# Stanford-ILIAD/PantheonRL

Hardware: AMD Instinct MI355X
Metric: env-steps/sec (all agents) Overcooked-simple PPO self-play (higher is better)
Workload: dtype f32; 1 GPU; OvercookedMultiEnv-v0 layout=simple, PPO self-play (two independent PPO learners per GPU), synthetic (n_envs, n_steps, obs_dim) rollouts; n_envs=1024, n_steps=128, obs_dim=62, features=62, n_logits=6, batch_size=32768, n_epochs=10, agents_per_gpu=2, parallelism=2 agent(s) per gpu x1 gpu(s) = 2 learners (single process), launch_mode=graph, gemm_mode=2, action_masks=none, rollout=scripted, rollout_requested=scripted

## Files before the change

include/pantheon_hip.h:

```cpp
#ifndef PANTHEON_HIP_H
#define PANTHEON_HIP_H

#ifdef __cplusplus
extern "C" {
#endif

#define PH_ABI_VERSION 7
#define PH_HIDDEN 64
#define PH_MAX_COMP 256
#define PH_MAX_LOGITS 64
#define PH_MAX_BOX_ACT 16
#define PH_NSTAT 8
#define PH_MOD_MAX 8
#define PH_MAX_RANKS 16

#define PH_SPACE_BOX 0
#define PH_SPACE_DISCRETE 1

typedef struct ph_ctx ph_ctx;

typedef struct ph_space {
  int kind;
  int n;
  int nvec[PH_MAX_COMP];
// ... 8 lines not shown
  int D;
  int F;
  int A;
  int L;
  int P;
  int pi_W1, pi_b1, pi_W2, pi_b2, vf_W1, vf_b1, vf_W2, vf_b2, act_W, act_b, val_W, val_b;
} ph_layout;

typedef struct ph_rollout {
  int T, E;
  float *observations;
  float *actions;
  float *rewards;
  float *episode_starts;
  float *values;
  float *log_probs;
  float *advantages;
  float *returns;
} ph_rollout;

typedef struct ph_ppo_hyper {
  float learning_rate;
  float clip_range;
  float clip_range_vf;
  float ent_coef;
  float vf_coef;
  float max_grad_norm;
  float target_kl;
  int normalize_advantage;
  float adam_beta1, adam_beta2, adam_eps;
} ph_ppo_hyper;

typedef struct ph_opt_state {
  float *params;
  float *adam_m;
  float *adam_v;
  int *step;
} ph_opt_state;

int ph_abi_version(void);
const char *ph_last_error(void);
int ph_device_count(int *n_out );
int ph_ctx_create(int device, ph_ctx **out );
int ph_ctx_destroy(ph_ctx *ctx);
int ph_ctx_set_stream(ph_ctx *ctx, void *hip_stream );
int ph_ctx_sync(ph_ctx *ctx);
int ph_graph_begin(ph_ctx *ctx);
int ph_graph_end(ph_ctx *ctx, int *graph_id_out );
int ph_graph_launch(ph_ctx *ctx, int graph_id);
int ph_ctx_set_rng_epoch(ph_ctx *ctx, unsigned long long *epoch_dev );
int ph_rng_epoch_advance(ph_ctx *ctx);
int ph_debug_set_profile_buffer(ph_ctx *ctx, long long *stamps_dev);
int ph_debug_weight_image_mismatches(ph_ctx *ctx, const ph_spec *spec, const float *params, int *mismatches);
int ph_set_exclusive_device(ph_ctx *ctx, int exclusive);
int ph_ctx_step_errors(ph_ctx *ctx, unsigned int *count_out );
int ph_timer_start(ph_ctx *ctx);
int ph_timer_stop(ph_ctx *ctx, float *ms_out );

int ph_layout_of(const ph_spec *spec , ph_layout *out );
int ph_debug_split_tables(const ph_spec *spec, int *slab_map, int *image_map, int *eligible);
int ph_debug_split_oh_tables(const ph_spec *spec, int *slab_map, int *image_map, int *slab_len_out, int *image_elems_out,
                             int *eligible);

int ph_buffer_add(ph_ctx *ctx, const ph_spec *spec, const ph_rollout *rb, int pos, const float *obs ,
                  const float *actions , const float *episode_start ,
                  const float *values , const float *log_probs );
int ph_buffer_add_reward(ph_ctx *ctx, const ph_rollout *rb, int pos, const float *reward ,
                         const unsigned char *env_mask );
int ph_buffer_add_reward_const(ph_ctx *ctx, const ph_rollout *rb, int pos, float reward);
#define PH_JOINT_MATCH_BONUS 0
#define PH_JOINT_RPS 1
int ph_ctx_set_joint_reward_rule(ph_ctx *ctx, int rule);

int ph_buffer_add_reward_joint(ph_ctx *ctx, const ph_rollout *rb, int pos, const float *base_reward ,
                               const int *joint_actions, int n_seats, int seat, const int *partner_seat ,
                               float bonus);
int ph_roundrobin_env_step(ph_ctx *ctx, const int *joint_actions, int *partnerid, const float *base_reward,
                           const float *done, float *reward_out, int *alt_action_out, float *next_block, int block_ld,
                           int n_partners, float bonus, int n);
typedef struct ph_rr_link {
  int n_partners, rank;
  int n, block_ld;
  void *area[PH_MAX_RANKS];
  unsigned long long *error;
  unsigned long long timeout_cycles;
} ph_rr_link;
typedef struct ph_rr_ego {
  const ph_spec *spec;
  const float *params;
  const float *obs_seq;
  const float *base_reward_seq;
  const float *done_seq;
  float *blocks;
  int *partnerid;
  float *rewards;
  int *alt_actions;
  int *partner_trace;
  const float *episode_start0;
  unsigned long long seed, counter0;
  float *values, *log_probs;
  const ph_rollout *rb;
  float bonus;
} ph_rr_ego;
typedef struct ph_rr_partner {
  const ph_spec *spec;
  const float *params;
// ... 458 lines not shown
```

pantheonrl_amd/_native.py:

```python
from __future__ import annotations

import ctypes as C
import os
from typing import Optional, Sequence

PH_HIDDEN = 64
PH_MAX_COMP = 256
PH_MAX_LOGITS = 64
PH_MAX_BOX_ACT = 16
PH_NSTAT = 8
PH_SPACE_BOX = 0
PH_SPACE_DISCRETE = 1
STAT_NAMES = ("policy_loss", "value_loss", "entropy_loss", "clip_fraction", "approx_kl", "loss", "grad_norm", "applied")

_HERE = os.path.dirname(os.path.abspath(__file__))
LIB_PATH = os.environ.get("PANTHEON_HIP_LIB") or os.path.join(_HERE, "csrc", "libpantheon_hip.so")


class NativeError(RuntimeError):
    """Raised for any non-zero status from the C ABI (message from ph_last_error)."""


class PhSpace(C.Structure):
    _fields_ = [("kind", C.c_int), ("n", C.c_int), ("nvec", C.c_int * PH_MAX_COMP)]
# ... 160 lines not shown
                ("alt_values", C.c_void_p), ("alt_log_probs", C.c_void_p), ("alt_pos", C.c_void_p),
                ("alt_boundary", C.c_void_p), ("alt_term", C.c_void_p), ("alt_open", C.c_void_p), ("alt_acted", C.c_void_p),
                ("alt_seed", C.c_ulonglong),
                ("obs_ego", C.c_void_p), ("obs_alt", C.c_void_p), ("episodes", C.c_void_p),
                ("es_alt", C.c_void_p), ("running", C.c_void_p), ("can", C.c_void_p), ("done", C.c_void_p)]


PH_BLOCK_STATE_WORDS = 12

PH_MAX_POOL = 8
PH_POOL_LEARNER, PH_POOL_FROZEN, PH_POOL_SCRIPTED = 0, 1, 2
POOL_RESAMPLE = {"robin": 0, "random": 1}


class PhPoolMember(C.Structure):
    _fields_ = [("kind", C.c_int), ("params", C.c_void_p), ("rb", C.POINTER(PhRollout)), ("pos", C.c_void_p),
                ("boundary", C.c_void_p), ("term", C.c_void_p), ("open", C.c_void_p), ("values", C.c_void_p),
                ("log_probs", C.c_void_p), ("seed", C.c_ulonglong)]


class PhLiarPool(C.Structure):
    _fields_ = [("n", C.c_int), ("spec", C.POINTER(PhSpec)),
                ("hands", C.c_void_p), ("history", C.c_void_p), ("nmoves", C.c_void_p), ("ego_first", C.c_void_p),
                ("dice_seed", C.c_ulonglong), ("probegostart", C.c_float),
                ("ego_params", C.c_void_p), ("ego_rb", C.POINTER(PhRollout)), ("ego_actions", C.c_void_p),
                ("ego_values", C.c_void_p), ("ego_log_probs", C.c_void_p), ("ego_episode_start", C.c_void_p),
                ("ego_seed", C.c_ulonglong),
                ("members", C.POINTER(PhPoolMember)), ("n_members", C.c_int), ("partnerid", C.c_void_p),
                ("resample", C.c_int), ("pool_seed", C.c_ulonglong),
                ("alt_actions", C.c_void_p), ("alt_acted", C.c_void_p),
                ("obs_ego", C.c_void_p), ("obs_alt", C.c_void_p), ("episodes", C.c_void_p),
                ("obs_next", C.c_void_p), ("rew1", C.c_void_p), ("rew2", C.c_void_p), ("es_alt", C.c_void_p),
                ("done1", C.c_void_p), ("done2", C.c_void_p), ("running", C.c_void_p), ("can", C.c_void_p),
                ("alt_opens", C.c_void_p), ("ego_opens", C.c_void_p), ("done", C.c_void_p)]

SIGNATURES = {
    "ph_abi_version": [],
    "ph_roundrobin_env_step": [_vp, _vp, _vp, _vp, _vp, _vp, _vp, _vp, _i, _i, C.c_float, _i],
    "ph_last_error": [],
    "ph_device_count": [C.POINTER(_i)],
    "ph_ctx_create": [_i, C.POINTER(_vp)],
    "ph_ctx_destroy": [_vp],
    "ph_ctx_set_stream": [_vp, _vp],
    "ph_ctx_sync": [_vp],
    "ph_graph_begin": [_vp],
    "ph_graph_end": [_vp, C.POINTER(_i)],
    "ph_graph_launch": [_vp, _i],
    "ph_ctx_set_rng_epoch": [_vp, _vp],
    "ph_rng_epoch_advance": [_vp],
    "ph_debug_set_profile_buffer": [_vp, _vp],
    "ph_set_exclusive_device": [_vp, _i],
    "ph_ctx_step_errors": [_vp, C.POINTER(C.c_uint)],
    "ph_debug_weight_image_mismatches": [_vp, C.POINTER(PhSpec), _vp, C.POINTER(C.c_int)],
    "ph_timer_start": [_vp],
    "ph_timer_stop": [_vp, C.POINTER(C.c_float)],
    "ph_layout_of": [C.POINTER(PhSpec), C.POINTER(PhLayout)],
    "ph_debug_split_tables": [C.POINTER(PhSpec), C.POINTER(C.c_int), C.POINTER(C.c_int), C.POINTER(C.c_int)],
    "ph_debug_split_oh_tables": [C.POINTER(PhSpec), _vp, _vp, C.POINTER(_i), C.POINTER(_i), C.POINTER(_i)],
    "ph_buffer_add": [_vp, C.POINTER(PhSpec), C.POINTER(PhRollout), _i, _vp, _vp, _vp, _vp, _vp],
    "ph_buffer_add_reward": [_vp, C.POINTER(PhRollout), _i, _vp, _vp],
    "ph_buffer_add_reward_joint": [_vp, C.POINTER(PhRollout), _i, _vp, _vp, _i, _i, _vp, C.c_float],
    "ph_buffer_reset": [_vp, C.POINTER(PhSpec), C.POINTER(PhRollout)],
    "ph_gae": [_vp, C.POINTER(PhRollout), _vp, _vp, _d, _d, _i],
    "ph_policy_forward": [_vp, C.POINTER(PhSpec), _vp, _vp, _i, _vp, _vp, _vp, _ull, _ull, _i, _vp, _vp, _vp, _vp, _vp,
                          _vp, C.POINTER(PhRollout), _i, _vp, _vp, _i],
    "ph_ctx_set_joint_reward_rule": [_vp, _i],
    "ph_adapmult_layout_of": [C.POINTER(PhSpec), _i, _vp],
    "ph_adapmult_forward": [_vp, C.POINTER(PhSpec), _i, _vp, _vp, _i, _vp, _vp, _vp, _ull, _ull, _i, _vp, _vp, _vp, _vp, _vp,
                            _vp, C.POINTER(PhRollout), _i, _vp],
    "ph_adapmult_minibatch_grad": [_vp, C.POINTER(PhSpec), _i, _vp, C.POINTER(PhRollout), C.POINTER(PhPpoHyper), _vp, _i, _vp, _vp,
                                   _vp],
    "ph_adapmult_train": [_vp, C.POINTER(PhSpec), _i, C.POINTER(PhOptState), C.POINTER(PhRollout), C.POINTER(PhPpoHyper), _i, _i,
                          _vp, _ull, _vp, _vp],
    "ph_policy_act_host": [_vp, C.POINTER(PhSpec), _vp, _vp, _i, _vp, _ull, _ull, _i, _vp, _vp, _vp, C.POINTER(PhRollout), _i, _i],
    "ph_buffer_add_reward_const": [_vp, C.POINTER(PhRollout), _i, C.c_float],
    "ph_policy_step_multi": [_vp, _i, C.POINTER(PhStepCall)],
    "ph_policy_forward_ragged": [_vp, C.POINTER(PhSpec), _vp, _vp, _vp, _ull, _ull, _i, _vp, _vp, _vp, C.POINTER(PhRollout),
                                 _vp, _vp, _vp],
    "ph_buffer_add_reward_ragged": [_vp, C.POINTER(PhRollout), _vp, _vp, _vp],
    "ph_ragged_advance": [_vp, C.POINTER(PhRollout), _vp, _vp],
    "ph_buffer_compact_columns": [_vp, C.POINTER(PhSpec), C.POINTER(PhRollout), C.POINTER(PhRollout), _vp, _i],
    "ph_fix_illegal_actions": [_vp, _vp, _vp, _i, _i],
    "ph_rps_step": [_vp, _vp, _vp, _vp, _vp, _i],
    "ph_liar_step": [_vp, _vp, _vp, _vp, _vp, _vp, _vp, _vp, _vp, _vp, _i],
    "ph_liar_reset": [_vp, _vp, _vp, _vp, _vp, _vp, _ull, _ull, C.c_float, _i],
    "ph_liar_obs": [_vp, _vp, _vp, _vp, _vp, _vp, _vp, _i],
    "ph_liar_selfplay_step": [_vp, C.POINTER(PhLiarSelfPlay), _i, _ull, _i],
    "ph_liar_selfplay_rollout": [_vp, C.POINTER(PhLiarSelfPlay), _i, _i, _ull],
    "ph_pool_forward": [_vp, C.POINTER(PhSpec), C.POINTER(PhPoolMember), _i, _vp, _vp, _vp, _ull, _vp, _vp, _i],
    "ph_liar_default_actions": [_vp, _vp, _vp, _vp, _i],
    "ph_liar_pool_step": [_vp, C.POINTER(PhLiarPool), _i, _ull, _i],
    "ph_block_reset": [_vp, _i, _vp, _vp, _ull, _ull, _i],
    "ph_block_step": [_vp, _i, _vp, _vp, _i, _vp, _vp, _vp, _vp, _i],
    "ph_block_obs": [_vp, _i, _vp, _i, _vp, _vp, _i],
    "ph_block_selfplay_step": [_vp, C.POINTER(PhBlockSelfPlay), _i, _ull],
    "ph_block_replay_host": [_i, _i, _i, _vp, _vp, _vp, _vp, _vp, _vp, _vp, _i, _ull, _ull, _i],
    "ph_framestack_push": [_vp, _vp, _vp, _vp, _vp, _i, _i, _i],
    "ph_scripted_rollout": [_vp, C.POINTER(PhSpec), _vp, _vp, _vp, _vp, _i, _i, _vp, _ull, _ull, _vp, _vp, _vp,
                            C.POINTER(PhRollout), _i, _i],
    "ph_ppo_train": [_vp, C.POINTER(PhSpec), C.POINTER(PhOptState), C.POINTER(PhRollout), C.POINTER(PhPpoHyper), _i, _i,
                     _vp, _ull, _vp, _i],
    "ph_ppo_train_multi": [C.POINTER(PhTrainCall), _i],
    "ph_comm_unique_id": [_vp],
    "ph_comm_init": [_vp, _vp, _i, _i],
    "ph_comm_destroy": [_vp],
    "ph_all_gather_i32": [_vp, _vp, _vp, _i],
# ... 233 lines not shown
```

pantheonrl_amd/csrc/ph_abi.hip:

```cpp
#include <dlfcn.h>
#include <hip/hip_runtime.h>
#include <rccl/rccl.h>

#include <atomic>
#include <chrono>
#include <cmath>
#include <cstdio>
#include <cstdint>
#include <cstring>
#include <mutex>
#include <string>
#include <vector>

#include "ph_launch.h"
#include "ph_block.h"
#include "ph_arch.h"
#include "ph_pool.h"

namespace ph {

namespace {
struct LdsGrant {
  const void* kernel;
  int device;
// ... 75 lines not shown
}

struct ph_ctx {
  int device = 0;
  hipStream_t stream = nullptr;
  float* slabs = nullptr;
  size_t slabs_cap = 0;
  float* statpart = nullptr;
  size_t statpart_cap = 0;
  float* grad = nullptr;
  size_t grad_cap = 0;
  float* blocksq = nullptr;
  size_t blocksq_cap = 0;
  float* advstats = nullptr;
  size_t advstats_cap = 0;
  ph::AdamBias* adam_bias = nullptr;
  size_t adam_bias_cap = 0;
  float* act_stage_host = nullptr;
  float* act_stage_dev = nullptr;
  size_t act_stage_cap = 0;
  unsigned int* act_done_host = nullptr;
  unsigned int* act_done_dev = nullptr;
  unsigned int act_seq = 0;
  unsigned int* fwd_host_done = nullptr;
  int joint_reward_rule = 0;
  int wimage_zeroed_for = 0;
  size_t wimage_cap = 0;
  bool exclusive = false;
  unsigned short* wimage = nullptr;
  double* advpart = nullptr;
  size_t advpart_cap = 0;
  int* perm_idx = nullptr;
  size_t perm_idx_cap = 0;
  int* perm_phys = nullptr;
  size_t perm_phys_cap = 0;
  uint4* ximg = nullptr;
  size_t ximg_cap = 0;
  uint4* rec_pi = nullptr;
  uint4* rec_vf = nullptr;
  size_t rec_cap = 0;
  uint4* rowrec = nullptr;
  size_t rowrec_cap = 0;
  unsigned long long* step_words = nullptr;
  size_t step_words_cap = 0;
  unsigned int* step_gen = nullptr;
  float* am_buf = nullptr;
  size_t am_buf_cap = 0;
  float* adap_extra = nullptr;
  size_t adap_extra_cap = 0;
  float* adap_loss = nullptr;
  size_t adap_loss_cap = 0;
  float* scalars = nullptr;
  int* stop_flag = nullptr;
  std::vector<SpecCache> specs;
  std::vector<hipGraphExec_t> graphs;
  bool capturing = false;
  hipEvent_t ev0 = nullptr, ev1 = nullptr;
  ph_p2p* p2p_dev = nullptr;
  ph_p2p p2p_host;
  bool p2p_valid = false;
  void* comm = nullptr;
  int comm_world = 1, comm_rank = 0;
  hipEvent_t ev_grad = nullptr;
  int num_cu = 256;
  int exchange_blocks_per_cu = 0;
  unsigned long long* rng_epoch = nullptr;
  ph::PoolMemberDev* pool_dev = nullptr;
  ph::PoolMemberDev pool_host[PH_MAX_POOL];
  int pool_count = 0;
  int* pool_order = nullptr;
  size_t pool_order_cap = 0;
  int* pool_tiles = nullptr;
  size_t pool_tiles_cap = 0;
  long long* prof = nullptr;
  struct ModWs {
    float* act = nullptr;
    size_t act_cap = 0;
    int* maps = nullptr;
    ph_spec spec;
    ph_modular mod;
    bool maps_valid = false;
    float* kl_sum = nullptr;
    int* scratch = nullptr;
  } mw;
};

namespace {

struct DevGuard {
  int prev = -1;
  bool switched = false;
  explicit DevGuard(const ph_ctx* ctx) {
    if (!ctx) return;
    if (hipGetDevice(&prev) == hipSuccess && prev != ctx->device) switched = hipSetDevice(ctx->device) == hipSuccess;
  }
  ~DevGuard() {
    if (switched) (void)hipSetDevice(prev);
  }
  DevGuard(const DevGuard&) = delete;
  DevGuard& operator=(const DevGuard&) = delete;
};

template <typename T>
int ensure(const ph_ctx* ctx, T*& p, size_t& cap, size_t n) {
  if (n <= cap) return 0;
  if (ctx->capturing) return fail("workspace would grow inside graph capture: run the same call once outside capture first");
// ... 534 lines not shown
  if (!ctx) return fail("null ctx");
  if (ctx->capturing) return fail("already capturing");
  if (ctx->stream == nullptr) return fail("graph capture needs a non-default stream (ph_ctx_set_stream)");
  PH_HIP(hipStreamBeginCapture(ctx->stream, hipStreamCaptureModeRelaxed));
  ctx->capturing = true;
  return 0;
}

int ph_graph_end(ph_ctx* ctx, int* graph_id_out) {
  DevGuard dev_guard(ctx);
  if (!ctx || !graph_id_out) return fail("null ctx/graph_id_out");
  if (!ctx->capturing) return fail("not capturing");
  ctx->capturing = false;
  hipGraph_t g = nullptr;
  PH_HIP(hipStreamEndCapture(ctx->stream, &g));
  hipGraphExec_t ge = nullptr;
  hipError_t e = hipGraphInstantiate(&ge, g, nullptr, nullptr, 0);
  (void)hipGraphDestroy(g);
  if (e != hipSuccess) return fail_hip("hipGraphInstantiate", e);
  ctx->graphs.push_back(ge);
  *graph_id_out = (int)ctx->graphs.size() - 1;
  return 0;
}

int ph_graph_launch(ph_ctx* ctx, int graph_id) {
  DevGuard dev_guard(ctx);
  if (!ctx) return fail("null ctx");
  if (graph_id < 0 || graph_id >= (int)ctx->graphs.size()) return fail("bad graph id");
  PH_HIP(hipGraphLaunch(ctx->graphs[graph_id], ctx->stream));
  return 0;
}

int ph_ctx_set_rng_epoch(ph_ctx* ctx, unsigned long long* epoch_dev) {
  DevGuard dev_guard(ctx);
  if (!ctx) return fail("null ctx");
  ctx->rng_epoch = epoch_dev;
  return 0;
}
int ph_rng_epoch_advance(ph_ctx* ctx) {
  DevGuard dev_guard(ctx);
  if (!ctx) return fail("null ctx");
  if (!ctx->rng_epoch) return fail("ph_rng_epoch_advance: no epoch word attached");
  PH_HIP(ph::launch_epoch_advance(ctx->rng_epoch, ctx->stream));
  return 0;
}

int ph_debug_set_profile_buffer(ph_ctx* ctx, long long* stamps_dev) {
  DevGuard dev_guard(ctx);
  if (!ctx) return fail("null ctx");
  ctx->prof = stamps_dev;
  return 0;
}

int ph_debug_weight_image_mismatches(ph_ctx* ctx, const ph_spec* spec, const float* params, int* mismatches_host) {
  DevGuard dev_guard(ctx);
  if (!ctx || !params || !mismatches_host) return fail("ph_debug_weight_image_mismatches: null argument");
  ph::NetDims nd;
  if (resolve(ctx, spec, &nd)) return 1;
  *mismatches_host = -1;
  if (!ctx->wimage || !nd.wimage_map) return 0;
  int* d = nullptr;
  PH_HIP(hipMalloc((void**)&d, sizeof(int)));
  PH_HIP(hipMemsetAsync(d, 0, sizeof(int), ctx->stream));
  PH_HIP(ph::launch_weight_image_check(params, ctx->wimage, nd.wimage_map, nd.lay.P, d, ctx->stream));
  PH_HIP(hipMemcpyAsync(mismatches_host, d, sizeof(int), hipMemcpyDeviceToHost, ctx->stream));
  PH_HIP(hipStreamSynchronize(ctx->stream));
  (void)hipFree(d);
  return 0;
}

int ph_set_exclusive_device(ph_ctx* ctx, int exclusive) {
  if (!ctx) return fail("null ctx");
  ctx->exclusive = exclusive != 0;
  return 0;
}

int ph_ctx_step_errors(ph_ctx* ctx, unsigned int* count_out) {
  DevGuard dev_guard(ctx);
  if (!ctx || !count_out) return fail("ph_ctx_step_errors: null argument");
  *count_out = 0u;
  if (!ctx->step_gen) return 0;
  PH_HIP(hipMemcpyAsync(count_out, ctx->step_gen + 1, sizeof(unsigned int), hipMemcpyDeviceToHost, ctx->stream));
  PH_HIP(hipStreamSynchronize(ctx->stream));
  return 0;
}

int ph_timer_start(ph_ctx* ctx) {
  DevGuard dev_guard(ctx);
  if (!ctx) return fail("null ctx");
  PH_HIP(hipEventRecord(ctx->ev0, ctx->stream));
  return 0;
}
int ph_timer_stop(ph_ctx* ctx, float* ms_out) {
  DevGuard dev_guard(ctx);
  if (!ctx || !ms_out) return fail("null ctx/ms_out");
  PH_HIP(hipEventRecord(ctx->ev1, ctx->stream));
  PH_HIP(hipEventSynchronize(ctx->ev1));
  PH_HIP(hipEventElapsedTime(ms_out, ctx->ev0, ctx->ev1));
  return 0;
}

int ph_layout_of(const ph_spec* spec, ph_layout* out) { return layout_of(spec, out); }

int ph_debug_split_tables(const ph_spec* spec, int* slab_map , int* image_map , int* eligible) {
  if (!spec || !slab_map || !image_map || !eligible) return fail("ph_debug_split_tables: null argument");
  ph_layout lay;
// ... 1591 lines not shown
    for (int k = 0; k < n_calls; ++k) {
      if (mbi >= total[k]) continue;
      hipStream_t s = t[k].ctx->stream;
      if (prev && prev_stream != s) PH_HIP(hipStreamWaitEvent(s, prev, 0));
      MbPlan pl;
      if (train_launch_grad(t[k], mbi, &pl)) return 1;
      PH_HIP(hipEventRecord(t[k].ctx->ev_grad, s));
      prev = t[k].ctx->ev_grad;
      prev_stream = s;
      if (train_launch_step(t[k], mbi, pl)) return 1;
    }
  }
  return 0;
}

namespace {
int minibatch_grad_run(const char* who, ph_ctx* ctx, const ph_spec* spec, const float* params, const ph_rollout* rb,
                       const ph_ppo_hyper* hp, const int* indices, int nb, float* grad_out, float* stats_out, int gemm_mode,
                       const ph_adap_loss* adap, const ph_arch* arch = nullptr);
}

int ph_ppo_minibatch_grad(ph_ctx* ctx, const ph_spec* spec, const float* params, const ph_rollout* rb,
                          const ph_ppo_hyper* hp, const int* indices, int nb, float* grad_out, float* stats_out,
                          int gemm_mode) {
  DevGuard dev_guard(ctx);
  return minibatch_grad_run("ph_ppo_minibatch_grad", ctx, spec, params, rb, hp, indices, nb, grad_out, stats_out, gemm_mode, nullptr);
}

int ph_adap_minibatch_grad(ph_ctx* ctx, const ph_spec* spec, const float* params, const ph_rollout* rb,
                           const ph_ppo_hyper* hp, const int* indices, int nb, float* grad_out, float* stats_out,
                           int gemm_mode, const ph_adap_loss* adap) {
  DevGuard dev_guard(ctx);
  if (!adap) return fail("ph_adap_minibatch_grad: null context-term description");
  return minibatch_grad_run("ph_adap_minibatch_grad", ctx, spec, params, rb, hp, indices, nb, grad_out, stats_out, gemm_mode, adap);
}

namespace {
int minibatch_grad_run(const char* who, ph_ctx* ctx, const ph_spec* spec, const float* params, const ph_rollout* rb,
                       const ph_ppo_hyper* hp, const int* indices, int nb, float* grad_out, float* stats_out, int gemm_mode,
                       const ph_adap_loss* adap, const ph_arch* arch) {
  if (check_minibatch_call(who, ctx, params, rb, hp, indices, nb, grad_out)) return 1;
  ph::NetDims nd;
  ph::ArchDims ad;
  if (arch) {
    if (arch_resolve(ctx, spec, arch, &nd, &ad)) return 1;
  } else {
    if (resolve(ctx, spec, &nd, adap == nullptr)) return 1;
    select_gemm(nd, gemm_mode);
  }
  const int P = nd.lay.P;
  const MbPlan pl = plan_minibatch(ctx, nd, nb, arch ? &ad : nullptr);
  if (ensure_train_ws(ctx, P, slab_len_of(nd), pl.nwg, 1, 0, (size_t)nb)) return 1;
  hipStream_t s = ctx->stream;
  PH_HIP(ph::launch_set_int(ctx->stop_flag, 0, s));
  if (rebuild_weight_image(ctx, nd, params)) return 1;
  if (build_grad_pack(ctx, nd, rb, (size_t)nb)) return 1;
  ph::AdvStatArgs aa = adv_args_minibatch(ctx, rb, indices, nb);
  fill_adv_records(aa, ctx, nd, rb);
  PH_HIP(ph::launch_adv_stats(aa, 1, s));
  ph::GradArgs g;
  std::memset(&g, 0, sizeof(g));
  fill_grad_args(g, nd, params, rb, hp, ctx);
  g.idx = indices;
  g.idx_phys = ctx->perm_phys;
  g.nb = nb;
  g.advstats = ctx->advstats;
  g.ntiles = pl.ntiles;
  if (arch) PH_HIP(ph::launch_arch_grad(g, ad, pl.nwg, gemm_mode, s));
  else PH_HIP(ph::launch_ppo_grad(g, pl.nwg, gemm_mode, s));
  ph::ReduceArgs r = reduce_args(ctx, hp, nullptr, P, slab_len_of(nd), nd.slab_map, pl.nwg, nb, grad_out, stats_out);
  if (adap) {
    if (adap_check(ctx, nd, adap, who)) return 1;
    if (adap_launch(ctx, nd, params, rb, adap, indices, nb, 0, &r)) return 1;
  }
  PH_HIP(ph::launch_ppo_reduce(r, s));
  return 0;
}
}

int ph_arch_layout_of(const ph_spec* spec, const ph_arch* arch, ph_arch_layout* out) { return arch_layout(spec, arch, out); }

int ph_arch_lds_bytes(const ph_spec* spec, const ph_arch* arch, int* grad_bytes_out, int* grad_rows_out, int* fwd_bytes_out) {
  ph::ArchDims ad;
  ph::NetDims nd;
  if (arch_host_dims(spec, arch, &nd, &ad)) return 1;
  const int R = ph::arch_grad_rows(nd, ad);
  if (grad_bytes_out) *grad_bytes_out = (int)ph::arch_grad_lds_bytes(nd, ad, R);
  if (grad_rows_out) *grad_rows_out = R;
  if (fwd_bytes_out) *fwd_bytes_out = (int)ph::arch_fwd_lds_bytes(nd, ad);
  return 0;
}

int ph_arch_fits(const ph_spec* spec, const ph_arch* arch) {
  ph::ArchDims ad;
  ph::NetDims nd;
  if (arch_host_dims(spec, arch, &nd, &ad)) return 1;
  return arch_lds_refusal(nd, ad);
}

int ph_arch_forward(ph_ctx* ctx, const ph_spec* spec, const ph_arch* arch, const float* params, const float* obs, int n,
                    const unsigned char* action_mask, const float* uniforms, const float* given_actions,
                    unsigned long long seed, unsigned long long counter, int deterministic, int* actions_i32,
                    float* actions_f32, float* values, float* log_probs, float* entropy, float* logits,
                    const ph_rollout* rb, int pos, const float* episode_start_in, const float* pending_reward, int gemm_mode) {
  DevGuard dev_guard(ctx);
  if (!arch) return fail("null arch/layout");
  return forward_run("ph_arch_forward", ctx, spec, arch, params, obs, n, action_mask, uniforms, given_actions, seed, counter,
// ... 902 lines not shown
```

pantheonrl_amd/csrc/ph_ppo_split.hip:

```cpp
#include "ph_split_tile.h"


namespace ph {

struct SplitRowMeta {
  int phys;
  float adv, old, act;
};

struct XRows {
  uint4 v[6];
  __device__ __forceinline__ void issue(int physv, const uint4* ximg, int zero_row, int lane) {
#pragma unroll
    for (int i = 0; i < 2; ++i) {
      const int r = 8 * i + (lane >> 3);
      int p = __builtin_amdgcn_ds_bpermute(4 * r, physv);
      p = p < 0 ? zero_row : p;
      const uint4* src = ximg + (size_t)p * XIMG_ROW_U4 + (lane & 7);
#pragma unroll
      for (int q = 0; q < 3; ++q) v[i * 3 + q] = ld_nt16(src + q * 8);
    }
  }
  __device__ __forceinline__ void commit(char* x, int wave, int lane) const {
#pragma unroll
    for (int i = 0; i < 2; ++i) {
      const int row = 16 * wave + 8 * i + (lane >> 3);
      const int off = row * PL_ROW + (((lane & 7) ^ pl_swz(row)) << 4);
#pragma unroll
      for (int q = 0; q < 3; ++q) *reinterpret_cast<uint4*>(x + off + q * PL_BYTES) = v[i * 3 + q];
    }
  }
};

template <int NK, bool FOLD>
__global__ __launch_bounds__(256, 2) void ppo_grad_split_kernel(GradArgs a) {
  const int stop_now = __builtin_nontemporal_load(a.stop_flag);
  PH_STAMP(a.prof, 0);
  extern __shared__ __attribute__((aligned(16))) float smem_f[];
  char* smem = reinterpret_cast<char*>(smem_f);
  constexpr int R = 64;
  constexpr int DZ_ROW = 3 * PL_ROW, DZ_PL = PL_ROW;
  constexpr int XT = 0, H1T = PB_BYTES, DZ2 = 2 * PB_BYTES;
  const NetDims& nd = a.nd;
  const ph_layout& lay = nd.lay;
  auto h2_swz = [](int r) -> int { return (r & 1) | ((r & 2) ? 12 : 0); };
  auto h2_at = [&](int r, int gran) -> float* { return reinterpret_cast<float*>(smem + DZ2 + r * DZ_ROW + ((gran ^ h2_swz(r)) << 4)); };
  float* hw = smem_f + 3 * PB_BYTES / 4;
  float* dzs = hw + HW_FLOATS;
  float* b1s = dzs + R * 8;
  float* b2s = b1s + HID;
  float* hbs = b2s + HID;
  float* radv = hbs + 16;
  float* rold = radv + R;
  float* ract = rold + R;
  int* rowphys = (int*)(ract + R);

  const int net = blockIdx.y;
  const int oB1 = net == 0 ? lay.pi_b1 : lay.vf_b1, oB2 = net == 0 ? lay.pi_b2 : lay.vf_b2;
  const float inv_nb = 1.0f / (float)a.nb;
  const int nk = nd.L;

  const bool norm = net == 0 && a.norm_adv && a.nb > 1;
  const float* advp = a.advstats ? a.advstats : a.params;
  const float adv0 = __builtin_nontemporal_load(advp), adv1 = __builtin_nontemporal_load(advp + 1);
  const float adv_mean = norm ? adv0 : 0.f;
  const float adv_den = norm ? adv1 + 1e-8f : 1.f;

  const uint4* recs = net == 0 ? a.rec_pi : a.rec_vf;
  auto row_record = [&](int tile, int wave, int lane) -> SplitRowMeta {
    const int gi = tile * R + wave * 16 + lane;
    SplitRowMeta m;
    m.phys = -1;
    m.adv = m.old = m.act = 0.f;
    if (lane < 16 && gi < a.nb) {
      const uint4 r = ld_nt16(recs + gi);
      m.phys = (int)r.x;
      m.adv = __uint_as_float(r.y);
      m.old = __uint_as_float(r.z);
      m.act = __uint_as_float(r.w);
    }
    return m;
  };

  Frag3 W1f[2];
  XRows xt;
  SplitRowMeta meta;
  {
    const int tid = threadIdx.x, wave = tid >> 6, lane = tid & 63;
    meta = row_record(blockIdx.x, wave, lane);
    __builtin_amdgcn_sched_barrier(0);
    float bias1 = 0.f, bias2 = 0.f, hv0 = 0.f, hv1 = 0.f, hb = 0.f;
    if (tid < HID) {
      bias1 = a.params[oB1 + tid];
      bias2 = a.params[oB2 + tid];
    }
    if (net == 0) {
      const int j0 = tid >> 3, k = tid & 7;
      if (k < nk) {
        hv0 = a.params[lay.act_W + j0 * nk + k];
        hv1 = a.params[lay.act_W + (j0 + 32) * nk + k];
      }
      if (tid < 8) hb = (tid < nk) ? a.params[lay.act_b + tid] : -3.0e38f;
    } else {
      if (tid < HID) hv0 = a.params[lay.val_W + tid];
      if (tid == 0) hb = a.params[lay.val_b];
    }
    __builtin_amdgcn_sched_barrier(0);
    PH_STAMP(a.prof, 8);
    PH_STAMP(a.prof, 9);
    xt.issue(meta.phys, a.ximg, a.ximg_zero_row, lane);
    __builtin_amdgcn_sched_barrier(0);
    PH_STAMP(a.prof, 10);
    if (stop_now) return;
    PH_STAMP(a.prof, 11);
    if (tid < HID) {
      b1s[tid] = bias1;
      b2s[tid] = bias2;
    }
    if (net == 0) {
      hw[head_row(tid >> 3) + (tid & 7)] = hv0;
      hw[head_row((tid >> 3) + 32) + (tid & 7)] = hv1;
      if (tid < 8) hbs[tid] = hb;
    } else {
      if (tid < HID) hw[tid] = hv0;
      if (tid == 0) hbs[0] = hb;
    }
  }

  f32x4 gW1[4], gW2[4];
  f32x4 gB1 = {0.f, 0.f, 0.f, 0.f}, gB2 = {0.f, 0.f, 0.f, 0.f};
#pragma unroll
  for (int b = 0; b < 4; ++b) {
    gW1[b] = (f32x4){0.f, 0.f, 0.f, 0.f};
    gW2[b] = (f32x4){0.f, 0.f, 0.f, 0.f};
  }
  float gh0 = 0.f;
  float ghr[NK];
#pragma unroll
  for (int k = 0; k < NK; ++k) ghr[k] = 0.f;
  float ghb = 0.f;
  float st[NSTATP];
#pragma unroll
  for (int k = 0; k < NSTATP; ++k) st[k] = 0.f;

  float* const rslab = a.slabs + ((size_t)blockIdx.x * 2 + net) * RS_NET;
  bool slabs_out = false;
  bool first = true;
  int tile = blockIdx.x;
  do {
    int tidv = threadIdx.x;
    asm volatile("" : "+v"(tidv));
    const int tid = tidv, lane = tid & 63, wave = tid >> 6;
    const SplitSel ssel = split_sel();
    const int j = lane & 15, kg = lane >> 4;
    const bool has_next = tile + (int)gridDim.x < a.ntiles;
    const int unit = 16 * wave + j;

    {
      const uint4* img = reinterpret_cast<const uint4*>(a.wimage) + (size_t)((net * 4 + wave) * 18) * 64 + lane;
#pragma unroll
      for (int c = 0; c < 2; ++c)
#pragma unroll
        for (int p = 0; p < 3; ++p) W1f[c].p[p] = __builtin_bit_cast(bf16x8, img[(c * 3 + p) * 64]);
    }
    if (lane < 16) {
      const int row = wave * 16 + lane;
      rowphys[row] = meta.phys;
      radv[row] = (norm && meta.phys >= 0) ? (meta.adv - adv_mean) / adv_den : meta.adv;
      rold[row] = meta.old;
      ract[row] = meta.act;
    }
    if (first) PH_STAMP(a.prof, 14);
    xt.commit(smem + XT, wave, lane);
    if (first) PH_STAMP(a.prof, 15);
    lds_barrier();
    if (first) PH_STAMP(a.prof, 1);

    const int pb0 = plain_base(j, kg, 0), pb1 = plain_base(j, kg, 1);
    int trb[4], csb[4];
    {
      const int a0 = 8 * kg + (j >> 2);
      const int g0 = ((j & 3) >> 1) ^ pl_swz(a0), row0 = a0 * PL_ROW + 8 * (j & 1);
      const int g1 = (kg >> 1) ^ pl_swz(unit), row1 = unit * PL_ROW + 8 * (kg & 1);
#pragma unroll
      for (int k = 0; k < 4; ++k) {
        trb[k] = row0 + ((g0 ^ (2 * k)) << 4);
        csb[k] = row1 + ((g1 ^ (2 * k)) << 4);
      }
    }
    auto ld_trf = [&](int buf, int c, int mblk) -> Frag3 {
      return ld_tr(smem, trb[mblk], trb[mblk ^ 1], buf + 32 * c * PL_ROW, buf + (32 * c + 4) * PL_ROW);
    };

    f32x4 d1[4];
    Frag3 W2f[2];
    {
      const uint4* img = reinterpret_cast<const uint4*>(a.wimage) + (size_t)((net * 4 + wave) * 18 + 6) * 64 + lane;
#pragma unroll
      for (int c = 0; c < 2; ++c)
#pragma unroll
        for (int p = 0; p < 3; ++p) W2f[c].p[p] = __builtin_bit_cast(bf16x8, img[(c * 3 + p) * 64]);
    }
    {
      const float bb = FOLD ? 0.f : b1s[unit];
      Frag3 xa = ld_plain(smem, pb0, XT), xb = ld_plain(smem, pb1, XT);
#pragma unroll
      for (int b = 0; b < 4; ++b) {
        f32x4 acc = {0.f, 0.f, 0.f, 0.f};
        acc = mma6(xa, W1f[0], acc);
        acc = mma6(xb, W1f[1], acc);
        if (b < 3) {
          xa = ld_plain(smem, pb0, XT + (b + 1) * 16 * PL_ROW);
          xb = ld_plain(smem, pb1, XT + (b + 1) * 16 * PL_ROW);
        }
        float v[4];
#pragma unroll
        for (int r = 0; r < 4; ++r) {
          v[r] = fast_tanh(FOLD ? acc[r] : acc[r] + bb);
          d1[b][r] = 1.0f - v[r] * v[r];
        }
        asm volatile("" : "+v"(v[0]), "+v"(v[1]), "+v"(v[2]), "+v"(v[3]) : "v"(d1[b][0]), "v"(d1[b][1]), "v"(d1[b][2]), "v"(d1[b][3]));
        bf16x4 p[3];
        split4(ssel, v, p);
        st_planes4(smem, H1T + csb[b], p);
      }
    }
    lds_barrier();
    if (first) PH_STAMP(a.prof, 2);

    SplitRowMeta meta_next = meta;
    if (has_next) meta_next = row_record(tile + gridDim.x, wave, lane);
    {
      const float4 bb = *reinterpret_cast<const float4*>(b2s + 16 * wave + 4 * kg);
      Frag3 xa = ld_trf(H1T, 0, 0), xb = ld_trf(H1T, 1, 0);
#pragma unroll
      for (int b = 0; b < 4; ++b) {
        f32x4 acc = {0.f, 0.f, 0.f, 0.f};
        acc = mma6(W2f[0], xa, acc);
        acc = mma6(W2f[1], xb, acc);
        if (b < 3) {
          xa = ld_trf(H1T, 0, b + 1);
          xb = ld_trf(H1T, 1, b + 1);
        }
        *reinterpret_cast<float4*>(h2_at(16 * b + j, 4 * wave + kg)) =
            make_float4(fast_tanh(acc[0] + bb.x), fast_tanh(acc[1] + bb.y), fast_tanh(acc[2] + bb.z), fast_tanh(acc[3] + bb.w));
      }
    }
    lds_barrier();
    if (first) PH_STAMP(a.prof, 3);

    float dzv[16];
    const int hr = tid >> 2, hq = tid & 3;
    {
      const int r = hr, q = hq;
      const bool valid = rowphys[r] >= 0;
      float h[16];
#pragma unroll
      for (int g = 0; g < 4; ++g) {
        const float4 v = *reinterpret_cast<const float4*>(h2_at(r, 2 * q + (g & 1) + 8 * (g >> 1)));
        h[4 * g] = v.x; h[4 * g + 1] = v.y; h[4 * g + 2] = v.z; h[4 * g + 3] = v.w;
      }
      if (net == 0) {
        float z[NK];
#pragma unroll
        for (int k = 0; k < NK; ++k) z[k] = 0.f;
        for_head_rows<NK>(hw, q, [&](int m, const float4& w0, const float4& w1) {
          const float wk[8] = {w0.x, w0.y, w0.z, w0.w, w1.x, w1.y, w1.z, w1.w};
#pragma unroll
          for (int k = 0; k < NK; ++k) z[k] = __builtin_fmaf(h[m], wk[k], z[k]);
        });
        float pr[NK];
        float mx = -3.0e38f;
#pragma unroll
        for (int k = 0; k < NK; ++k) {
          z[k] = quad_sum(z[k]) + hbs[k];
          mx = fmaxf(mx, z[k]);
        }
        float se = 0.f;
#pragma unroll
        for (int k = 0; k < NK; ++k) {
          pr[k] = fast_exp(z[k] - mx);
          se += pr[k];
        }
        const float lse = mx + fast_log(se), inv = __builtin_amdgcn_rcpf(se);
// ... 101 lines not shown
          const float dk[8] = {da[i].x, da[i].y, da[i].z, da[i].w, db[i].x, db[i].y, db[i].z, db[i].w};
#pragma unroll
          for (int k = 0; k < NK; ++k) ghr[k] = __builtin_fmaf(hv[i], dk[k], ghr[k]);
        }
        __builtin_amdgcn_sched_barrier(0);
      }
      if (lane < NK) ghb += lds_sum16(dzs + wave * 16 * 8 + lane, 8);
    } else {
      float hv[16], dv[16];
      const char* hrow = smem + DZ2 + wave * (16 * DZ_ROW);
      const float* drow = dzs + wave * 16;
      int col4[4];
#pragma unroll
      for (int i = 0; i < 4; ++i) col4[i] = ((((lane >> 2) ^ h2_swz(i)) << 2) | (lane & 3)) * 4;
#pragma unroll
      for (int i = 0; i < 16; ++i) {
        hv[i] = *reinterpret_cast<const float*>(hrow + i * DZ_ROW + col4[i & 3]);
        dv[i] = drow[i];
      }
      __builtin_amdgcn_sched_barrier(0);
#pragma unroll
      for (int i = 0; i < 16; ++i) {
        gh0 = __builtin_fmaf(hv[i], dv[i], gh0);
        ghb += dv[i];
      }
    }
    wave_lds_sync();

    {
      const int sw = pl_swz(hr);
#pragma unroll
      for (int g = 0; g < 2; ++g) {
        Frag3 f;
        split8(ssel, dzv + 8 * g, f);
        st_planes8<DZ_PL>(smem, DZ2 + hr * DZ_ROW + (((4 * g + hq) ^ sw) << 4), f);
      }
    }
    lds_barrier();
    if (first) PH_STAMP(a.prof, 5);

    f32x4 dh1[4];
    {
      const int a0 = 8 * kg + (j >> 2), g0 = ((j & 3) >> 1) ^ pl_swz(a0), row0 = a0 * DZ_ROW + 8 * (j & 1);
      const int tlo = row0 + ((g0 ^ (2 * wave)) << 4), thi = row0 + ((g0 ^ (2 * (wave ^ 1))) << 4);
      const int db0 = j * DZ_ROW + ((kg ^ pl_swz(j)) << 4), db1 = j * DZ_ROW + (((4 + kg) ^ pl_swz(j)) << 4);
      Frag3 W2b[2];
      {
        const uint4* img = reinterpret_cast<const uint4*>(a.wimage) + (size_t)((net * 4 + wave) * 18 + 12) * 64 + lane;
#pragma unroll
        for (int c = 0; c < 2; ++c)
#pragma unroll
          for (int p = 0; p < 3; ++p) W2b[c].p[p] = __builtin_bit_cast(bf16x8, img[(c * 3 + p) * 64]);
      }
#pragma unroll
      for (int c = 0; c < 2; ++c) {
        const Frag3 dz = ld_tr<DZ_PL>(smem, tlo, thi, DZ2 + 32 * c * DZ_ROW, DZ2 + (32 * c + 4) * DZ_ROW);
        gB2 = mma_ones(dz, gB2);
#pragma unroll
        for (int b = 0; b < 4; ++b) {
          const Frag3 h1 = ld_plain(smem, c == 0 ? pb0 : pb1, H1T + b * 16 * PL_ROW);
          gW2[b] = mma6(h1, dz, gW2[b]);
        }
      }
      if (!has_next) {
        float* const w2o = rslab + RS_W2 + (wave * 4 * 64 + lane) * 4;
        st_slab16<0>(w2o, gW2[0]);
        st_slab16<1024>(w2o, gW2[1]);
        st_slab16<2048>(w2o, gW2[2]);
        st_slab16<3072>(w2o, gW2[3]);
        if (lane < 16) rslab[RS_B2 + 16 * wave + lane] = gB2[0];
      }
#pragma unroll
      for (int b = 0; b < 4; ++b) {
        f32x4 acc = {0.f, 0.f, 0.f, 0.f};
#pragma unroll
        for (int c = 0; c < 2; ++c)
          acc = mma6(ld_plain<DZ_PL>(smem, c == 0 ? db0 : db1, DZ2 + b * 16 * DZ_ROW), W2b[c], acc);
#pragma unroll
        for (int r = 0; r < 4; ++r) dh1[b][r] = acc[r] * d1[b][r];
      }
    }
    lds_barrier();
    if (first) PH_STAMP(a.prof, 6);

#pragma unroll
    for (int b = 0; b < 4; ++b) {
      float v[4] = {dh1[b][0], dh1[b][1], dh1[b][2], dh1[b][3]};
      bf16x4 p[3];
      split4(ssel, v, p);
      st_planes4(smem, H1T + csb[b], p);
    }
    wave_lds_sync();

    meta = meta_next;
    if (has_next) xt.issue(meta.phys, a.ximg, a.ximg_zero_row, lane);
    {
      const Frag3 dz0 = ld_plain(smem, pb0, H1T + wave * 16 * PL_ROW);
      const Frag3 dz1 = ld_plain(smem, pb1, H1T + wave * 16 * PL_ROW);
      if constexpr (!FOLD) {
        gB1 = mma_ones(dz0, gB1);
        gB1 = mma_ones(dz1, gB1);
      }
      float* const w1o = rslab + RS_W1 + (wave * 4 * 64 + lane) * 4;
#pragma unroll
      for (int b = 0; b < 4; ++b) {
        gW1[b] = mma6(ld_trf(XT, 0, b), dz0, gW1[b]);
        gW1[b] = mma6(ld_trf(XT, 1, b), dz1, gW1[b]);
        if (!has_next) {
          if (b == 0) st_slab16<0>(w1o, gW1[0]);
          else if (b == 1) st_slab16<1024>(w1o, gW1[1]);
          else if (b == 2) st_slab16<2048>(w1o, gW1[2]);
          else st_slab16<3072>(w1o, gW1[3]);
        }
      }
      if (!has_next) {
        if constexpr (!FOLD)
          if (lane < 16) rslab[RS_B1 + 16 * wave + lane] = gB1[0];
        slabs_out = true;
      }
    }
    lds_barrier();
    if (first) PH_STAMP(a.prof, 7);
    tile += gridDim.x;
    first = false;
  } while (tile < a.ntiles);
  PH_STAMP(a.prof, 12);

  {
    const int tid = threadIdx.x, lane = tid & 63, wave = tid >> 6;
    if (!slabs_out) {
      float* const w2o = rslab + RS_W2 + (wave * 4 * 64 + lane) * 4;
      float* const w1o = rslab + RS_W1 + (wave * 4 * 64 + lane) * 4;
      st_slab16<0>(w2o, gW2[0]); st_slab16<1024>(w2o, gW2[1]); st_slab16<2048>(w2o, gW2[2]); st_slab16<3072>(w2o, gW2[3]);
      st_slab16<0>(w1o, gW1[0]); st_slab16<1024>(w1o, gW1[1]); st_slab16<2048>(w1o, gW1[2]); st_slab16<3072>(w1o, gW1[3]);
      if (lane < 16) {
        rslab[RS_B2 + 16 * wave + lane] = gB2[0];
        if constexpr (!FOLD) rslab[RS_B1 + 16 * wave + lane] = gB1[0];
      }
    }
#pragma unroll
    for (int k = 0; k < NSTATP; ++k) {
      float v = st[k];
#pragma unroll
      for (int off = 32; off > 0; off >>= 1) v += __shfl_down(v, off, 64);
      st[k] = v;
    }
    float* part = smem_f;
    part[(0 * 4 + wave) * 64 + lane] = gh0;
    part[(1 * 4 + wave) * 64 + lane] = ghb;
    if (lane == 0) {
#pragma unroll
      for (int k = 0; k < NSTATP; ++k) part[(2 * 4 + wave) * 64 + k] = st[k];
    }
    if (net == 0) {
#pragma unroll
      for (int k = 0; k < NK; ++k) part[((3 + k) * 4 + wave) * 64 + lane] = ghr[k];
    }
    lds_barrier();
    auto wsum = [&](int which, int idx) {
      return ((part[(which * 4 + 0) * 64 + idx] + part[(which * 4 + 1) * 64 + idx]) + part[(which * 4 + 2) * 64 + idx]) +
             part[(which * 4 + 3) * 64 + idx];
    };
    if (net == 1 && tid < HID) rslab[RS_HW + tid] = wsum(0, tid);
    if (net == 0) {
#pragma unroll
      for (int k0 = 0; k0 < NK; k0 += 4) {
        const int k = k0 + (tid >> 6), jj = tid & 63;
        if (k < NK) rslab[RS_HW + jj * 8 + k] = wsum(3 + k, jj);
      }
    }
    if (net == 0 && tid < 8) rslab[RS_HB + tid] = wsum(1, tid);
    if (net == 1 && tid == 0) rslab[RS_HB] = wsum(1, 0);
    if (tid < NSTATP) a.statpart[((size_t)net * gridDim.x + blockIdx.x) * NSTATP + tid] = wsum(2, tid);
  }
  PH_STAMP(a.prof, 13);
}

static size_t grad_split_lds_bytes() {
  return (size_t)3 * PB_BYTES + sizeof(float) * (size_t)(HW_FLOATS + 64 * 8 + 2 * HID + 16 + 3 * 64 + 64);
}

bool grad_split_eligible(const NetDims& nd) {
  static int enabled = -1;
  if (enabled < 0) {
    const char* e = getenv("PH_GRAD_SPLIT");
    enabled = (e && e[0] == '0') ? 0 : 1;
  }
  return enabled && grad_fast_eligible(nd) && nd.obs_kind == PH_SPACE_BOX;
}

template <int NK, bool FOLD>
static hipError_t launch_split_inst(const GradArgs& a, int nwg, hipStream_t s) {
  const size_t lds = grad_split_lds_bytes();
  if (const hipError_t e = allow_dynamic_lds((const void*)ppo_grad_split_kernel<NK, FOLD>, lds); e != hipSuccess) return e;
  hipLaunchKernelGGL((ppo_grad_split_kernel<NK, FOLD>), dim3(nwg, 2), dim3(256), lds, s, a);
  return hipGetLastError();
}
template <int NK>
static hipError_t launch_split_nk(const GradArgs& a, int nwg, hipStream_t s) {
  return grad_fast_fold(a.nd) ? launch_split_inst<NK, true>(a, nwg, s) : launch_split_inst<NK, false>(a, nwg, s);
// ... 72 lines not shown
```

Baseline: 125.9 million agent-steps/s.

## Peel last tile of split PPO backward loop and make record loads branchless

The persistent tile loop in the split PPO backward kernel now breaks before the layer-1 weight-gradient stage and runs a peeled final iteration. Both the W2 and W1 slab stores move out of per-iteration has_next branches into that peeled tail, which drains outstanding vector-memory operations first. Row-record and parameter loads become unconditional clamped loads with selects instead of divergent branches, and a sched_barrier is added. The intent is to cut branch and VGPR pressure in the steady-state loop. It also adds debug hooks for the stop flag and grad slab copies, and moves the partial-sum scratch area to an LDS offset, which risks conflicts with the LDS layout if that offset is wrong.

```diff
diff --git a/include/pantheon_hip.h b/include/pantheon_hip.h
--- a/include/pantheon_hip.h
+++ b/include/pantheon_hip.h
@@ -84,6 +84,8 @@
 int ph_rng_epoch_advance(ph_ctx *ctx);
 int ph_debug_set_profile_buffer(ph_ctx *ctx, long long *stamps_dev);
 int ph_debug_weight_image_mismatches(ph_ctx *ctx, const ph_spec *spec, const float *params, int *mismatches);
+int ph_debug_hold_stop_flag(ph_ctx *ctx, int value);
+int ph_debug_copy_grad_slabs(ph_ctx *ctx, float *host_out, long long nfloats);
 int ph_set_exclusive_device(ph_ctx *ctx, int exclusive);
 int ph_ctx_step_errors(ph_ctx *ctx, unsigned int *count_out );
 int ph_timer_start(ph_ctx *ctx);
diff --git a/pantheonrl_amd/_native.py b/pantheonrl_amd/_native.py
--- a/pantheonrl_amd/_native.py
+++ b/pantheonrl_amd/_native.py
@@ -236,6 +236,8 @@
     "ph_set_exclusive_device": [_vp, _i],
     "ph_ctx_step_errors": [_vp, C.POINTER(C.c_uint)],
     "ph_debug_weight_image_mismatches": [_vp, C.POINTER(PhSpec), _vp, C.POINTER(C.c_int)],
+    "ph_debug_hold_stop_flag": [_vp, _i],
+    "ph_debug_copy_grad_slabs": [_vp, _vp, C.c_longlong],
     "ph_timer_start": [_vp],
     "ph_timer_stop": [_vp, C.POINTER(C.c_float)],
     "ph_layout_of": [C.POINTER(PhSpec), C.POINTER(PhLayout)],
diff --git a/pantheonrl_amd/csrc/ph_abi.hip b/pantheonrl_amd/csrc/ph_abi.hip
--- a/pantheonrl_amd/csrc/ph_abi.hip
+++ b/pantheonrl_amd/csrc/ph_abi.hip
@@ -151,6 +151,7 @@
   size_t adap_loss_cap = 0;
   float* scalars = nullptr;
   int* stop_flag = nullptr;
+  int debug_stop = 0;
   std::vector<SpecCache> specs;
   std::vector<hipGraphExec_t> graphs;
   bool capturing = false;
@@ -791,6 +792,21 @@
   return 0;
 }
 
+int ph_debug_hold_stop_flag(ph_ctx* ctx, int value) {
+  if (!ctx) return fail("null ctx");
+  ctx->debug_stop = value ? 1 : 0;
+  return 0;
+}
+
+int ph_debug_copy_grad_slabs(ph_ctx* ctx, float* host_out, long long nfloats) {
+  DevGuard dev_guard(ctx);
+  if (!ctx || !host_out || nfloats < 0) return fail("ph_debug_copy_grad_slabs: bad argument");
+  if (!ctx->slabs || (size_t)nfloats > ctx->slabs_cap) return fail("ph_debug_copy_grad_slabs: more floats than the context's slabs hold");
+  PH_HIP(hipStreamSynchronize(ctx->stream));
+  PH_HIP(hipMemcpy(host_out, ctx->slabs, sizeof(float) * (size_t)nfloats, hipMemcpyDeviceToHost));
+  return 0;
+}
+
 int ph_debug_weight_image_mismatches(ph_ctx* ctx, const ph_spec* spec, const float* params, int* mismatches_host) {
   DevGuard dev_guard(ctx);
   if (!ctx || !params || !mismatches_host) return fail("ph_debug_weight_image_mismatches: null argument");
@@ -2488,7 +2504,7 @@
   const MbPlan pl = plan_minibatch(ctx, nd, nb, arch ? &ad : nullptr);
   if (ensure_train_ws(ctx, P, slab_len_of(nd), pl.nwg, 1, 0, (size_t)nb)) return 1;
   hipStream_t s = ctx->stream;
-  PH_HIP(ph::launch_set_int(ctx->stop_flag, 0, s));
+  PH_HIP(ph::launch_set_int(ctx->stop_flag, ctx->debug_stop, s));
   if (rebuild_weight_image(ctx, nd, params)) return 1;
   if (build_grad_pack(ctx, nd, rb, (size_t)nb)) return 1;
   ph::AdvStatArgs aa = adv_args_minibatch(ctx, rb, indices, nb);
diff --git a/pantheonrl_amd/csrc/ph_ppo_split.hip b/pantheonrl_amd/csrc/ph_ppo_split.hip
--- a/pantheonrl_amd/csrc/ph_ppo_split.hip
+++ b/pantheonrl_amd/csrc/ph_ppo_split.hip
@@ -1,7 +1,11 @@
+#include <type_traits>
+
 #include "ph_split_tile.h"
 
 
 namespace ph {
+
+__device__ __forceinline__ void vm_drain() { __builtin_amdgcn_s_waitcnt(0x0F70); }
 
 struct SplitRowMeta {
   int phys;
@@ -68,17 +72,14 @@
 
   const uint4* recs = net == 0 ? a.rec_pi : a.rec_vf;
   auto row_record = [&](int tile, int wave, int lane) -> SplitRowMeta {
-    const int gi = tile * R + wave * 16 + lane;
+    const int gi = tile * R + wave * 16 + (lane & 15);
+    const uint4 r = ld_nt16(recs + (gi < a.nb ? gi : a.nb - 1));
+    const bool live = lane < 16 && gi < a.nb;
     SplitRowMeta m;
-    m.phys = -1;
-    m.adv = m.old = m.act = 0.f;
-    if (lane < 16 && gi < a.nb) {
-      const uint4 r = ld_nt16(recs + gi);
-      m.phys = (int)r.x;
-      m.adv = __uint_as_float(r.y);
-      m.old = __uint_as_float(r.z);
-      m.act = __uint_as_float(r.w);
-    }
+    m.phys = live ? (int)r.x : -1;
+    m.adv = live ? __uint_as_float(r.y) : 0.f;
+    m.old = live ? __uint_as_float(r.z) : 0.f;
+    m.act = live ? __uint_as_float(r.w) : 0.f;
     return m;
   };
 
@@ -89,21 +90,14 @@
     const int tid = threadIdx.x, wave = tid >> 6, lane = tid & 63;
     meta = row_record(blockIdx.x, wave, lane);
     __builtin_amdgcn_sched_barrier(0);
-    float bias1 = 0.f, bias2 = 0.f, hv0 = 0.f, hv1 = 0.f, hb = 0.f;
-    if (tid < HID) {
-      bias1 = a.params[oB1 + tid];
-      bias2 = a.params[oB2 + tid];
-    }
-    if (net == 0) {
-      const int j0 = tid >> 3, k = tid & 7;
-      if (k < nk) {
-        hv0 = a.params[lay.act_W + j0 * nk + k];
-        hv1 = a.params[lay.act_W + (j0 + 32) * nk + k];
-      }
-      if (tid < 8) hb = (tid < nk) ? a.params[lay.act_b + tid] : -3.0e38f;
-    } else {
-      if (tid < HID) hv0 = a.params[lay.val_W + tid];
-      if (tid == 0) hb = a.params[lay.val_b];
+    const int k7 = tid & 7, kc = k7 < nk ? k7 : nk - 1, u = tid & (HID - 1);
+    const float bias1 = a.params[oB1 + u], bias2 = a.params[oB2 + u];
+    float hv0 = a.params[net == 0 ? lay.act_W + (tid >> 3) * nk + kc : lay.val_W + u];
+    float hv1 = a.params[net == 0 ? lay.act_W + ((tid >> 3) + 32) * nk + kc : lay.val_W + u];
+    float hb = a.params[net == 0 ? lay.act_b + kc : lay.val_b];
+    if (net == 0 && k7 >= nk) {
+      hv0 = hv1 = 0.f;
+      hb = -3.0e38f;
     }
     __builtin_amdgcn_sched_barrier(0);
     PH_STAMP(a.prof, 8);
@@ -144,16 +138,45 @@
   for (int k = 0; k < NSTATP; ++k) st[k] = 0.f;
 
   float* const rslab = a.slabs + ((size_t)blockIdx.x * 2 + net) * RS_NET;
-  bool slabs_out = false;
   bool first = true;
   int tile = blockIdx.x;
-  do {
+  auto s7 = [&](auto last_tile, int wave, int lane) __attribute__((always_inline)) {
+    constexpr bool last = decltype(last_tile)::value;
+    const int j = lane & 15, kg = lane >> 4;
+    const int pb0 = plain_base(j, kg, 0), pb1 = plain_base(j, kg, 1);
+    const int a0 = 8 * kg + (j >> 2);
+    const int g0 = ((j & 3) >> 1) ^ pl_swz(a0), row0 = a0 * PL_ROW + 8 * (j & 1);
+    auto ld_trx = [&](int c, int mblk) -> Frag3 {
+      return ld_tr(smem, row0 + ((g0 ^ (2 * mblk)) << 4), row0 + ((g0 ^ (2 * (mblk ^ 1))) << 4), XT + 32 * c * PL_ROW, XT + (32 * c + 4) * PL_ROW);
+    };
+    const Frag3 dz0 = ld_plain(smem, pb0, H1T + wave * 16 * PL_ROW);
+    const Frag3 dz1 = ld_plain(smem, pb1, H1T + wave * 16 * PL_ROW);
+    if constexpr (!FOLD) {
+      gB1 = mma_ones(dz0, gB1);
+      gB1 = mma_ones(dz1, gB1);
+    }
+    float* const w1o = rslab + RS_W1 + (wave * 4 * 64 + lane) * 4;
+#pragma unroll
+    for (int b = 0; b < 4; ++b) {
+      gW1[b] = mma6(ld_trx(0, b), dz0, gW1[b]);
+      gW1[b] = mma6(ld_trx(1, b), dz1, gW1[b]);
+      if constexpr (last) {
+        if (b == 0) st_slab16<0>(w1o, gW1[0]);
+        else if (b == 1) st_slab16<1024>(w1o, gW1[1]);
+        else if (b == 2) st_slab16<2048>(w1o, gW1[2]);
+        else st_slab16<3072>(w1o, gW1[3]);
+      }
+    }
+    if constexpr (last && !FOLD)
+      if (lane < 16) rslab[RS_B1 + 16 * wave + lane] = gB1[0];
+  };
+  for (;;) {
+    const bool has_next = tile + (int)gridDim.x < a.ntiles;
     int tidv = threadIdx.x;
     asm volatile("" : "+v"(tidv));
     const int tid = tidv, lane = tid & 63, wave = tid >> 6;
     const SplitSel ssel = split_sel();
     const int j = lane & 15, kg = lane >> 4;
-    const bool has_next = tile + (int)gridDim.x < a.ntiles;
     const int unit = 16 * wave + j;
 
     {
@@ -228,8 +251,7 @@
     lds_barrier();
     if (first) PH_STAMP(a.prof, 2);
 
-    SplitRowMeta meta_next = meta;
-    if (has_next) meta_next = row_record(tile + gridDim.x, wave, lane);
+    const SplitRowMeta meta_next = row_record(has_next ? tile + (int)gridDim.x : tile, wave, lane);
     {
       const float4 bb = *reinterpret_cast<const float4*>(b2s + 16 * wave + 4 * kg);
       Frag3 xa = ld_trf(H1T, 0, 0), xb = ld_trf(H1T, 1, 0);
@@ -437,6 +459,7 @@
 #pragma unroll
           for (int p = 0; p < 3; ++p) W2b[c].p[p] = __builtin_bit_cast(bf16x8, img[(c * 3 + p) * 64]);
       }
+      __builtin_amdgcn_sched_barrier(0);
 #pragma unroll
       for (int c = 0; c < 2; ++c) {
         const Frag3 dz = ld_tr<DZ_PL>(smem, tlo, thi, DZ2 + 32 * c * DZ_ROW, DZ2 + (32 * c + 4) * DZ_ROW);
@@ -446,14 +469,6 @@
           const Frag3 h1 = ld_plain(smem, c == 0 ? pb0 : pb1, H1T + b * 16 * PL_ROW);
           gW2[b] = mma6(h1, dz, gW2[b]);
         }
-      }
-      if (!has_next) {
-        float* const w2o = rslab + RS_W2 + (wave * 4 * 64 + lane) * 4;
-        st_slab16<0>(w2o, gW2[0]);
-        st_slab16<1024>(w2o, gW2[1]);
-        st_slab16<2048>(w2o, gW2[2]);
-        st_slab16<3072>(w2o, gW2[3]);
-        if (lane < 16) rslab[RS_B2 + 16 * wave + lane] = gB2[0];
       }
 #pragma unroll
       for (int b = 0; b < 4; ++b) {
@@ -477,52 +492,33 @@
     }
     wave_lds_sync();
 
+    if (!has_next) break;
     meta = meta_next;
-    if (has_next) xt.issue(meta.phys, a.ximg, a.ximg_zero_row, lane);
-    {
-      const Frag3 dz0 = ld_plain(smem, pb0, H1T + wave * 16 * PL_ROW);
-      const Frag3 dz1 = ld_plain(smem, pb1, H1T + wave * 16 * PL_ROW);
-      if constexpr (!FOLD) {
-        gB1 = mma_ones(dz0, gB1);
-        gB1 = mma_ones(dz1, gB1);
-      }
-      float* const w1o = rslab + RS_W1 + (wave * 4 * 64 + lane) * 4;
-#pragma unroll
-      for (int b = 0; b < 4; ++b) {
-        gW1[b] = mma6(ld_trf(XT, 0, b), dz0, gW1[b]);
-        gW1[b] = mma6(ld_trf(XT, 1, b), dz1, gW1[b]);
-        if (!has_next) {
-          if (b == 0) st_slab16<0>(w1o, gW1[0]);
-          else if (b == 1) st_slab16<1024>(w1o, gW1[1]);
-          else if (b == 2) st_slab16<2048>(w1o, gW1[2]);
-          else st_slab16<3072>(w1o, gW1[3]);
-        }
-      }
-      if (!has_next) {
-        if constexpr (!FOLD)
-          if (lane < 16) rslab[RS_B1 + 16 * wave + lane] = gB1[0];
-        slabs_out = true;
-      }
-    }
+    xt.issue(meta.phys, a.ximg, a.ximg_zero_row, lane);
+    s7(std::false_type{}, wave, lane);
     lds_barrier();
     if (first) PH_STAMP(a.prof, 7);
     tile += gridDim.x;
     first = false;
-  } while (tile < a.ntiles);
+  }
+  {
+    int tidv = threadIdx.x;
+    asm volatile("" : "+v"(tidv));
+    const int lane = tidv & 63, wave = tidv >> 6;
+    vm_drain();
+    float* const w2o = rslab + RS_W2 + (wave * 4 * 64 + lane) * 4;
+    st_slab16<0>(w2o, gW2[0]);
+    st_slab16<1024>(w2o, gW2[1]);
+    st_slab16<2048>(w2o, gW2[2]);
+    st_slab16<3072>(w2o, gW2[3]);
+    if (lane < 16) rslab[RS_B2 + 16 * wave + lane] = gB2[0];
+    s7(std::true_type{}, wave, lane);
+    if (first) PH_STAMP(a.prof, 7);
+  }
   PH_STAMP(a.prof, 12);
 
   {
     const int tid = threadIdx.x, lane = tid & 63, wave = tid >> 6;
-    if (!slabs_out) {
-      float* const w2o = rslab + RS_W2 + (wave * 4 * 64 + lane) * 4;
-      float* const w1o = rslab + RS_W1 + (wave * 4 * 64 + lane) * 4;
-      st_slab16<0>(w2o, gW2[0]); st_slab16<1024>(w2o, gW2[1]); st_slab16<2048>(w2o, gW2[2]); st_slab16<3072>(w2o, gW2[3]);
-      st_slab16<0>(w1o, gW1[0]); st_slab16<1024>(w1o, gW1[1]); st_slab16<2048>(w1o, gW1[2]); st_slab16<3072>(w1o, gW1[3]);
-      if (lane < 16) {
-        rslab[RS_B2 + 16 * wave + lane] = gB2[0];
-        if constexpr (!FOLD) rslab[RS_B1 + 16 * wave + lane] = gB1[0];
-      }
-    }
 #pragma unroll
     for (int k = 0; k < NSTATP; ++k) {
       float v = st[k];
@@ -530,7 +526,7 @@
       for (int off = 32; off > 0; off >>= 1) v += __shfl_down(v, off, 64);
       st[k] = v;
     }
-    float* part = smem_f;
+    float* part = smem_f + DZ2 / 4;
     part[(0 * 4 + wave) * 64 + lane] = gh0;
     part[(1 * 4 + wave) * 64 + lane] = ghb;
     if (lane == 0) {
```

New measurement: 124.8 million agent-steps/s. Within noise of the previous version (-0.9%).
